# waffcloud/sitewhere

Hardware: AMD Instinct MI355X
Metric: device_events_per_sec (higher is better)
Workload: dtype fp64/int64 (event values as in the reference; no reduced precision)

## Files before the change

### csrc/hip/swblock.h

```cpp
#pragma once
#include <hip/hip_runtime.h>
#include <stdint.h>
#include "swengine.h"

typedef unsigned long long ull;

__device__ __forceinline__ uint32_t lane_id() { return threadIdx.x & 63; }

template <typename T>
__device__ __forceinline__ T wave_incl_scan(T v) {
  const uint32_t lane = lane_id();
#pragma unroll
  for (int d = 1; d < 64; d <<= 1) {
    const T t = __shfl_up(v, d, 64);
    if (lane >= (uint32_t)d) v += t;
  }
  return v;
}

template <typename T, int WAVES = 4>
__device__ __forceinline__ T block_excl_scan(T v, T* total, T* lds) {
  const uint32_t wid = threadIdx.x >> 6;
  const T inc = wave_incl_scan(v);
  if (lane_id() == 63) lds[wid] = inc;
  __syncthreads();
  if (threadIdx.x == 0) {
    T acc = 0;
    for (int w = 0; w < WAVES; ++w) { const T t = lds[w]; lds[w] = acc; acc += t; }
    lds[WAVES] = acc;
  }
  __syncthreads();
  const T res = inc - v + lds[wid];
  *total = lds[WAVES];
  __syncthreads();
  return res;
}

template <int WAVES = 4>
__device__ __forceinline__ uint32_t block_sum_prefix(const uint32_t* v, int64_t k, uint32_t* lds) {
  uint32_t s = 0;
  for (int64_t i = threadIdx.x; i < k; i += WAVES * 64) s += v[i];
  uint32_t tot;
  block_excl_scan<uint32_t, WAVES>(s, &tot, lds);
  return tot;
}

template <bool BLOCK_WORDS>
__device__ __forceinline__ void step_snapshot_write(SwStepSnapshot* rec, uint32_t t, const uint32_t* scalars,
                                                    const uint32_t* block_meta, const uint32_t* rej_cnt,
                                                    const uint32_t* n_carry, bool produced) {
  constexpr uint32_t BLOCK = offsetof(SwStepSnapshot, block_bytes) / 4, CARRY = offsetof(SwStepSnapshot, n_carry) / 4,
                     REJ = offsetof(SwStepSnapshot, rej_refs) / 4, PAD = offsetof(SwStepSnapshot, pad) / 4;
  static_assert(BLOCK == SW_SC_WORDS && CARRY == BLOCK + 6 && REJ == CARRY + 2 && PAD == REJ + 2, "word ladder");
  uint32_t* w = reinterpret_cast<uint32_t*>(rec);
  if (t < BLOCK) w[t] = produced ? scalars[t] : 0u;
  else if (t < CARRY) { if (BLOCK_WORDS) w[t] = (produced && block_meta) ? block_meta[t - BLOCK] : 0u; }
  else if (t == CARRY || t == CARRY + 1) w[t] = n_carry ? n_carry[t - CARRY] : 0u;
  else if (t == REJ || t == REJ + 1) w[t] = (produced && rej_cnt) ? rej_cnt[t - REJ] : 0u;
}

extern "C" int sw_radix_sort_u32(uint32_t* keys, uint32_t* vals, const uint32_t* n_ptr, int64_t cap, int bits, uint32_t* hist,
                      uint32_t* vals_final, hipStream_t s);
```

### csrc/hip/swgpu.hip

```cpp
#include <hip/hip_runtime.h>
#include <hsa/hsa.h>
#include <hsa/hsa_ext_amd.h>
#include <stdint.h>
#include "swtypes.h"
#include "swdecode.h"
#include "swengine.h"
#include "swseg.h"
#include "swblock.h"

#define BLK 256
#define WAVES (BLK / 64)
#define TILE_ITEMS 4
#define TILE (BLK * TILE_ITEMS)
#define MAX_GRID 2048
#define STAGE_BYTES (32 * 1024)
#define MAX_PROBE 4096

#ifndef SW_XCD_REMAP
#define SW_XCD_REMAP 0
#endif
__device__ __forceinline__ uint32_t sw_block_id() {
#if SW_XCD_REMAP
  const uint32_t nwg = gridDim.x, orig = blockIdx.x, x = orig % 8u, q = nwg / 8u, r = nwg % 8u;
  return (x < r ? x * (q + 1u) : r * (q + 1u) + (x - r) * q) + orig / 8u;
// ... 2167 lines not shown

int sw_reject_pack(const void* recs, const int32_t* rej_idx, const uint8_t* status, const uint32_t* scalars,
                   int64_t cap, void* out, uint8_t* out_st, hipStream_t s) {
  static_assert(sizeof(SwEventRec) == 80, "k_reject_pack copies 5 x 16 B per record");
  if (cap <= 0 || cap > 0xffffffffll / 5) return -1;
  k_reject_pack<<<512, 256, 0, s>>>(reinterpret_cast<const uint4*>(recs), rej_idx, status, scalars, (uint32_t)cap,
                                    reinterpret_cast<uint4*>(out), out_st);
  return (int)hipGetLastError();
}

int sw_stream_wait_event(hipStream_t s, hipEvent_t e) { return (int)hipStreamWaitEvent(s, e, 0); }
int sw_event_record(hipEvent_t e, hipStream_t s) { return (int)hipEventRecord(e, s); }
int sw_memcpy_h2d_async(void* dst, const void* src, int64_t n, hipStream_t s) {
  return n > 0 ? (int)hipMemcpyAsync(dst, src, (size_t)n, hipMemcpyHostToDevice, s) : 0;
}
int sw_memset_async(void* dst, int32_t v, int64_t n, hipStream_t s) {
  return n > 0 ? (int)hipMemsetAsync(dst, v, (size_t)n, s) : 0;
}

int sw_step_snapshot(const uint32_t* scalars, const uint32_t* seg_meta, const uint32_t* rej_cnt,
                     const uint32_t* n_carry, int32_t produced, SwStepSnapshot* host, hipStream_t s) {
  k_step_snapshot<<<1, 64, 0, s>>>(scalars, seg_meta, rej_cnt, n_carry, produced, host);
  return (int)hipGetLastError();
}

int sw_frame_varint(const uint8_t* lens, int64_t nbytes, int64_t n_msgs, uint32_t* msg_off, uint32_t raw_bytes,
                    uint32_t* tmp, int64_t tmp_len, hipStream_t s) {
  int64_t nt = (nbytes + TILE - 1) / TILE;
  if (nt < 1) nt = 1;
  if (2 * nt > tmp_len) return -2;
  if (nbytes <= 0 || n_msgs <= 0) return (int)hipMemsetAsync(msg_off, 0, sizeof(uint32_t) * (n_msgs + 1), s);
  uint32_t* tcnt = tmp;
  uint32_t* tlen = tmp + nt;
  k_vlen_tiles<<<(unsigned)nt, BLK, 0, s>>>(lens, nbytes, tcnt, tlen);
  k_vlen_apply<<<(unsigned)nt, BLK, 0, s>>>(lens, nbytes, tcnt, tlen, msg_off, n_msgs, raw_bytes);
  return (int)hipGetLastError();
}

int sw_phase_decode(const SwEngineArgs* ap, hipStream_t s) {
  const SwEngineArgs a = *ap;
  if (a.n_msgs <= 0) {
    k_decode_begin<<<1, 64, 0, s>>>(a);
    (void)hipMemsetAsync(a.n_recs, 0, sizeof(uint32_t), s);
    return (int)hipGetLastError();
  }
  const unsigned nb = (unsigned)((a.n_msgs + BLK - 1) / BLK);
  k_decode_count<<<nb, BLK, 0, s>>>(a.raw, a.msg_off, a.n_msgs, a.msg_cnt, a.msg_evoff, a);
  k_decode_emit<<<nb, BLK, 0, s>>>(a);
  if (a.world > 1) k_decode_end<<<1, 64, 0, s>>>(a);
  return (int)hipGetLastError();
}

int sw_phase_partition(const SwEngineArgs* ap, hipStream_t s) {
  const SwEngineArgs a = *ap;
  const int64_t ntiles = (a.carry_cap + a.rec_cap + TILE - 1) / TILE;
  if (a.world > 64 || ntiles * a.world > a.part_tmp_len || !a.carry || !a.n_carry || !a.spill || !a.n_spill ||
      a.carry == a.spill || !a.part_owner || !a.part_bytes || !a.part_meta || ntiles >= 0x7fffffff)
    return -3;
  if (a.send_str && (!a.part_len || !a.carry_spans || !a.carry_str || !a.spill_spans || !a.spill_str ||
                     a.carry_str == a.spill_str || a.carry_str_cap <= 0 || a.carry_str_cap > 0xffffffffll ||
                     a.str_cap > 0x7fffffffll))
    return -4;
  k_part_count<<<(unsigned)ntiles, BLK, 0, s>>>(a.carry, a.n_carry, a.recs, a.n_recs, (int)a.world, (int)a.rank,
                                                a.part_tmp, ntiles, a);
  int rc = launch_scan(a.part_tmp, ntiles * a.world, a.part_tmp + ntiles * a.world, nullptr, a.scan_tmp,
                       a.scan_tmp_len, s);
  if (rc) return rc;
  const uint32_t* toff = a.part_tmp + ntiles * a.world;
  k_part_cut<<<(unsigned)a.world, BLK, 0, s>>>(toff, a.part_tmp, ntiles, a.n_carry, a.n_recs, a);
  k_part_write<<<(unsigned)ntiles, BLK, 0, s>>>(a.carry, a.n_carry, a.recs, a.n_recs, (int)a.world, (int)a.rank, toff,
                                                a.part_tmp, ntiles, a.send, a.shuf_cap, a.spill, a.carry_cap, a);
  k_part_counts<<<1, 64, 0, s>>>(toff, a.part_tmp, ntiles, (int)a.world, a);
  return (int)hipGetLastError();
}

int sw_phase_unpack(const SwEngineArgs* ap, hipStream_t s) {
  const SwEngineArgs a = *ap;
  if (a.work_str && (a.str_cap & 15)) return -5;
  k_unpack<<<grid_for(a.rec_cap), BLK, 0, s>>>(a.recv, a.recv_cnt, (int)a.world, a.shuf_cap, a.work, a.n_work,
                                               a.rec_cap, a);
  return (int)hipGetLastError();
}

__global__ void k_cl_prep(const uint32_t* __restrict__ ok_idx, const uint32_t* __restrict__ n_ok,
                          const int32_t* __restrict__ ev_asg, uint32_t* __restrict__ keys, uint32_t* __restrict__ vals) {
  const uint32_t n = *n_ok;
  for (int64_t j = (int64_t)BID * BLK + threadIdx.x; j < n; j += (int64_t)gridDim.x * BLK) {
    const uint32_t i = ok_idx[j];
    keys[j] = (uint32_t)ev_asg[i];
    vals[j] = i;
  }
}

__global__ __launch_bounds__(BLK) void k_ff_add_rows(SwEngineArgs a, const SwEventRec* __restrict__ R,
                                                     const uint32_t* __restrict__ idx,
                                                     const uint32_t* __restrict__ n_ptr, uint32_t cap) {
  if (!a.dd_ff) return;
  const uint32_t n = *n_ptr < cap ? *n_ptr : cap;
  uint32_t* __restrict__ t = a.dd_ff;
  const int gens = (int)a.dd_ff_gens, g = (int)a.dd_ff_meta[0];
  const int64_t bmask = a.dd_ff_bmask;
  const uint32_t lane = threadIdx.x & 63u, sub = lane & 3u, grp = lane >> 2;
  const ull gmask = 0xfull << (4u * grp);
  const int64_t g0 = ((int64_t)BID * BLK + threadIdx.x) >> 2;
  const int64_t gstride = ((int64_t)gridDim.x * BLK) >> 2;
  uint32_t dropped = 0;
  for (int64_t base = g0 - grp; base < (int64_t)n; base += gstride) {
    const int64_t j = base + grp;
    ull h = 0ull;
    if (j < (int64_t)n) h = R[idx ? idx[j] : (uint32_t)j].alt_hash;
    const ull m = sw_ff_mix(h);
    const uint32_t fp = sw_ff_fp(m);
    int64_t b = (int64_t)sw_ff_bucket(m, bmask);
    bool pending = h != 0ull;
    for (int p = 0; p < 2 * SW_FF_MAX_PROBE && __any(pending); ++p) {
      uint32_t* sl = t + (b * gens + g) * SW_FF_SLOTS;
      uint4 v = make_uint4(1u, 1u, 1u, 1u);
      if (pending) v = reinterpret_cast<const uint4*>(sl)[sub];
      const bool hit = pending && (v.x == fp || v.y == fp || v.z == fp || v.w == fp);
      if (__ballot(hit) & gmask) pending = false;
      const bool zero = pending && (!v.x || !v.y || !v.z || !v.w);
      const ull zb = __ballot(zero) & gmask;
      bool ok = false;
      if (pending && zb && lane == (uint32_t)(__ffsll((long long)zb) - 1)) {
        const int k = !v.x ? 0 : !v.y ? 1 : !v.z ? 2 : 3;
        const uint32_t old = atomicCAS(&sl[4u * sub + (uint32_t)k], 0u, fp);
        ok = old == 0u || old == fp;
      }
      if (__ballot(ok) & gmask) pending = false;
      else if (pending && !zb) b = (b + 1) & bmask;
    }
    if (pending && sub == 0u) ++dropped;
  }
  if (dropped) atomicAdd((ull*)&a.dd_ff_meta[5], (ull)dropped);
}

int sw_phase_process(const SwEngineArgs* ap, uint32_t* scratch4, hipStream_t s) {
  const SwEngineArgs a = *ap;
  const int g = grid_for(a.rec_cap);
  const int64_t ntiles = (a.rec_cap + TILE - 1) / TILE;
  if (2 * ntiles > a.scan_tmp_len) return -4;
  if (a.dd_ff && (a.dd_ff_gens < 2 || a.dd_ff_gens > SW_FF_MAX_GENS || !a.dd_ff_meta || a.dd_ff_bmask < 0))
    return -6;
  if (a.n_mtests < 0 || (a.n_mtests > 0 && (!a.mtests || a.n_tests + a.n_mtests > ZONE_LDS_TESTS))) return -7;
  k_lookup<<<g, BLK, 0, s>>>(a);
  if (a.dd_ff) k_ff_probe<<<g, BLK, 0, s>>>(a);
  k_dedup_claim<<<g, BLK, 0, s>>>(a);
  k_cmp_count<<<(unsigned)ntiles, BLK, 0, s>>>(a.status, a.n_work, a.cmp_tmp, ntiles, (ull*)a.stats, a.work,
                                               (const ull*)a.dd_key, a.dd_mask, a.seq_base, a.dd_meta,
                                               a.dd_ff, a.dd_ff_bmask, (int)a.dd_ff_gens, a.work_str ? -1 : (int)a.rank);
  k_cmp_write<<<(unsigned)ntiles, BLK, 0, s>>>(a.status, a.n_work, a.cmp_tmp, ntiles, a.ok_idx, a.rej_idx, a.n_ok,
                                               a.n_rej);
  int rc = 0;
  if (a.cl_bits > 0) {
    k_cl_prep<<<g, BLK, 0, s>>>(a.ok_idx, a.n_ok, a.ev_asg, a.cl_keys, a.cl_vals);
    rc = sw_radix_sort_u32(a.cl_keys, a.cl_vals, a.n_ok, a.rec_cap, (int)a.cl_bits, a.cl_hist, a.ok_idx, s);
    if (rc < 0) return rc;
  }
  const SwStrRef* wsp = a.world > 1 ? a.work_spans : a.spans;
  k_persist<<<g, BLK, 0, s>>>(a, a.work, a.ok_idx, a.ev_dev, a.ev_asg, a.n_ok, (uint32_t)a.rec_cap, wsp, nullptr);
  if (a.dd_ff) k_ff_add_rows<<<g, BLK, 0, s>>>(a, a.work, a.ok_idx, a.n_ok, (uint32_t)a.rec_cap);
  k_state_p2<<<g, BLK, 0, s>>>(a, a.n_ok, (uint32_t)a.rec_cap, nullptr);
  uint32_t* n_rule = scratch4;
  if (a.n_tests + a.n_mtests > 0) {
    const int64_t otiles = (a.rec_cap + TILE - 1) / TILE;
    ull* zmask = (ull*)a.zmask;
    uint32_t* ztile = a.ztile;
    if (a.n_tests > 0) {
      const size_t vtx_bytes = zone_vtx_in_lds(a) ? (size_t)a.n_zone_vtx * 2 * sizeof(double) : 0;
      k_zone_mask<<<(unsigned)otiles, BLK, vtx_bytes, s>>>(a, zmask, ztile);
    }
    if (a.n_mtests > 0) k_mx_mask<<<(unsigned)otiles, BLK, 0, s>>>(a, zmask, ztile, a.n_tests > 0 ? 0 : 1);
    k_zone_emit<<<(unsigned)otiles, BLK, 0, s>>>(a, zmask, ztile, n_rule);
  } else {
    k_gen_clamp<<<1, 64, 0, s>>>(a, n_rule);
  }
  k_presence<<<grid_for(a.n_asg), BLK, 0, s>>>(a);
  const int gg = grid_for(a.gen_cap);
  const uint32_t gcap = (uint32_t)a.gen_cap;
  k_intern_insert_list<<<gg, BLK, 0, s>>>(a.gen, a.n_gen, (ull*)a.nm_key, a.nm_id, a.nm_counter, a.nm_mask, gcap);
  k_persist<<<gg, BLK, 0, s>>>(a, a.gen, nullptr, a.gen_dev, a.gen_asg, a.n_gen, gcap, nullptr, a.n_ok);
  if (a.dd_ff) k_ff_add_rows<<<gg, BLK, 0, s>>>(a, a.gen, nullptr, a.n_gen, gcap);
  k_state_p2<<<gg, BLK, 0, s>>>(a, a.n_gen, gcap, a.n_ok);
  k_step_end<<<1, 64, 0, s>>>(a, n_rule);
  return (int)hipGetLastError();
}

__global__ void k_set_step_params(SwStepParams* sp, int64_t now_ms, int64_t batch_seq, int64_t presence_ms,
                                  SwOutRec* out, void* aux, int64_t raw_bytes) {
  if (threadIdx.x == 0 && BID == 0) {
    sp->now_ms = now_ms; sp->batch_seq = batch_seq; sp->presence_missing_ms = presence_ms; sp->out = out;
    sp->aux = aux; sp->raw_bytes = raw_bytes;
  }
}

__global__ void k_ff_add(uint32_t* t, int64_t bmask, int gens, int g, int64_t* meta, const ull* __restrict__ h,
                         int64_t n) {
  uint32_t dropped = 0;
  for (int64_t i = (int64_t)BID * BLK + threadIdx.x; i < n; i += (int64_t)gridDim.x * BLK)
    if (h[i] && !ff_add(t, bmask, gens, g, h[i])) ++dropped;
  if (dropped) atomicAdd((ull*)&meta[5], (ull)dropped);
}

__global__ void k_ff_clear(uint32_t* t, int64_t bmask, int gens, int g) { ff_clear_gen(t, bmask, gens, g); }

int sw_ff_add(void* tab, int64_t bmask, int64_t gens, int64_t gen, void* meta, const void* hashes, int64_t n,
              hipStream_t s) {
  if (n <= 0) return 0;
  if (gens < 2 || gens > SW_FF_MAX_GENS || gen < 0 || gen >= gens) return -2;
  const int64_t g = (n + BLK - 1) / BLK;
  k_ff_add<<<(unsigned)(g < 4096 ? g : 4096), BLK, 0, s>>>((uint32_t*)tab, bmask, (int)gens, (int)gen,
                                                          (int64_t*)meta, (const ull*)hashes, n);
  return (int)hipGetLastError();
}

int sw_ff_clear(void* tab, int64_t bmask, int64_t gens, int64_t g, hipStream_t s) {
  if (gens < 2 || gens > SW_FF_MAX_GENS || g < 0 || g >= gens) return -2;
  const int64_t nb = (bmask + 1) * 4;
  const int64_t gr = (nb + BLK - 1) / BLK;
  k_ff_clear<<<(unsigned)(gr < 8192 ? gr : 8192), BLK, 0, s>>>((uint32_t*)tab, bmask, (int)gens, (int)g);
  return (int)hipGetLastError();
}

int sw_set_step_params(SwStepParams* sp, int64_t now_ms, int64_t batch_seq, int64_t presence_ms, void* out,
                       void* aux, int64_t raw_bytes, hipStream_t s) {
  k_set_step_params<<<1, 64, 0, s>>>(sp, now_ms, batch_seq, presence_ms, (SwOutRec*)out, aux, raw_bytes);
  return (int)hipGetLastError();
}

int sw_graph_capture_process(const SwEngineArgs* ap, uint32_t* scratch4, int32_t with_unpack, hipStream_t s,
                             void** exec_out) {
  hipGraph_t g = nullptr;
  hipError_t e = hipStreamBeginCapture(s, hipStreamCaptureModeThreadLocal);
  if (e != hipSuccess) return 5000 + (int)e;
  int rc = 0;
  if (with_unpack) rc = sw_phase_unpack(ap, s);
  if (!rc) rc = sw_phase_process(ap, scratch4, s);
  e = hipStreamEndCapture(s, &g);
  if (rc) { if (g) (void)hipGraphDestroy(g); return rc; }
// ... 308 lines not shown
```

### csrc/hip/swindex.hip

```cpp
#include <hip/hip_runtime.h>
#include <stdint.h>
#include "swindex.h"
#include "swseg.h"
#include "swtypes.h"
#include "swblock.h"

#define RS_BLK 256
#define RS_ITEMS 16
#define RS_TILE (RS_BLK * RS_ITEMS)
#define RS_WAVES (RS_BLK / 64)

struct RsState {
  uint32_t* hist;
  uint32_t* off;
  uint32_t* tot;
};

__device__ __host__ __forceinline__ int64_t rs_tiles(int64_t cap) {
  const int64_t t = (cap + RS_TILE - 1) / RS_TILE;
  return t < 1 ? 1 : t;
}
__device__ __host__ __forceinline__ RsState rs_state(uint32_t* st, int64_t cap) {
  RsState r;
  const int64_t tiles = rs_tiles(cap);
  r.hist = st;
  r.off = st + tiles * 256;
  r.tot = r.off + tiles * 256;
  return r;
}

__global__ __launch_bounds__(RS_BLK) void k_rs_count(const uint32_t* __restrict__ keys, const uint32_t* __restrict__ n_ptr,
                                                     int shift, uint32_t mask, uint32_t* st_words, int64_t cap) {
  __shared__ uint32_t h[256];
  const RsState st = rs_state(st_words, cap);
  const uint32_t n = *n_ptr;
  const int64_t base = (int64_t)blockIdx.x * RS_TILE;
  if (base >= (int64_t)n) return;
  h[threadIdx.x] = 0;
  __syncthreads();
#pragma unroll
  for (int k = 0; k < RS_ITEMS; ++k) {
    const int64_t i = base + (int64_t)k * RS_BLK + threadIdx.x;
    if (i < (int64_t)n) atomicAdd(&h[(keys[i] >> shift) & mask], 1u);
  }
  __syncthreads();
  st.hist[(int64_t)blockIdx.x * 256 + threadIdx.x] = h[threadIdx.x];
}

__global__ __launch_bounds__(RS_BLK) void k_rs_offsets(const uint32_t* __restrict__ n_ptr, uint32_t* st_words, int64_t cap) {
  __shared__ uint32_t red[RS_WAVES + 1];
  const RsState st = rs_state(st_words, cap);
  const uint32_t n = *n_ptr;
  const int64_t ntiles = ((int64_t)n + RS_TILE - 1) / RS_TILE;
  const uint32_t d = blockIdx.x;
  uint32_t run = 0;
  for (int64_t t0 = 0; t0 < ntiles; t0 += RS_BLK) {
    const int64_t t = t0 + threadIdx.x;
    const uint32_t v = t < ntiles ? st.hist[t * 256 + d] : 0u;
    uint32_t tot;
    const uint32_t pre = block_excl_scan(v, &tot, red);
    if (t < ntiles) st.off[t * 256 + d] = run + pre;
    run += tot;
  }
  if (threadIdx.x == 0) st.tot[d] = run;
}

struct RsLds {
  uint32_t sk[RS_TILE];
  uint32_t sv[RS_TILE];
  uint32_t wc[RS_WAVES][256];
  uint32_t ls[256];
  uint32_t run[256];
  uint32_t gb[256];
  uint32_t red[RS_WAVES + 1];
};

__global__ __launch_bounds__(RS_BLK) void k_rs_scatter(const uint32_t* __restrict__ kin, const uint32_t* __restrict__ vin,
                                                       uint32_t* __restrict__ kout, uint32_t* __restrict__ vout,
                                                       const uint32_t* __restrict__ n_ptr, int shift, int dbits,
                                                       uint32_t* st_words, int64_t cap) {
  __shared__ RsLds L;
  const RsState st = rs_state(st_words, cap);
  const uint32_t n = *n_ptr;
  const int64_t tile = blockIdx.x;
  const int64_t base = tile * RS_TILE;
  if (base >= (int64_t)n) return;
  const uint32_t t = threadIdx.x, lane = lane_id(), wid = t >> 6;
  const uint32_t mask = (1u << dbits) - 1u;
  uint32_t K[RS_ITEMS], V[RS_ITEMS];
#pragma unroll
  for (int k = 0; k < RS_ITEMS; ++k) {
    const int64_t i = base + (int64_t)k * RS_BLK + t;
    const bool ok = i < (int64_t)n;
    K[k] = ok ? kin[i] : 0u;
    V[k] = ok ? vin[i] : 0u;
  }
  uint32_t gtot, ctot;
  const uint32_t gpre = block_excl_scan(t <= mask ? st.tot[t] : 0u, &gtot, L.red);
  const uint32_t c = t <= mask ? st.hist[tile * 256 + t] : 0u;
  L.ls[t] = block_excl_scan(c, &ctot, L.red);
  L.gb[t] = gpre + (t <= mask ? st.off[tile * 256 + t] : 0u);
  L.run[t] = 0;
#pragma unroll
  for (int w = 0; w < RS_WAVES; ++w) L.wc[w][t] = 0;
  __syncthreads();
  const ull lt = (1ull << lane) - 1ull;
#pragma unroll
  for (int k = 0; k < RS_ITEMS; ++k) {
    const int64_t i = base + (int64_t)k * RS_BLK + t;
    const bool valid = i < (int64_t)n;
    const uint32_t d = (K[k] >> shift) & mask;
    ull peers = __ballot(valid);
    for (int b = 0; b < dbits; ++b) {
      const bool bit = (d >> b) & 1u;
      const ull m = __ballot(valid && bit);
      peers &= bit ? m : ~m;
    }
    const uint32_t rank = (uint32_t)__popcll(peers & lt);
    if (valid && rank == 0) L.wc[wid][d] = (uint32_t)__popcll(peers);
    __syncthreads();
    if (valid) {
      uint32_t pos = L.ls[d] + L.run[d] + rank;
      for (uint32_t w = 0; w < wid; ++w) pos += L.wc[w][d];
      L.sk[pos] = K[k];
      L.sv[pos] = V[k];
    }
    __syncthreads();
    uint32_t add = 0;
#pragma unroll
    for (int w = 0; w < RS_WAVES; ++w) { add += L.wc[w][t]; L.wc[w][t] = 0; }
    L.run[t] += add;
    __syncthreads();
  }
  const uint32_t m = (uint32_t)(((int64_t)n - base) < RS_TILE ? (int64_t)n - base : RS_TILE);
  for (uint32_t i = t; i < m; i += RS_BLK) {
    const uint32_t key = L.sk[i];
    const uint32_t d = (key >> shift) & mask;
    const uint32_t pos = L.gb[d] + (i - L.ls[d]);
    kout[pos] = key;
    vout[pos] = L.sv[i];
  }
}

extern "C" {

int64_t sw_radix_tmp_words(int64_t cap) { return 2 * 256 * rs_tiles(cap) + 256 + 8; }

int sw_radix_sort_u32(uint32_t* keys, uint32_t* vals, const uint32_t* n_ptr, int64_t cap, int bits, uint32_t* state,
                      uint32_t* vals_final, hipStream_t s) {
  if (bits <= 0) return 0;
  if (bits > 32) bits = 32;
  const unsigned grid = (unsigned)rs_tiles(cap);
  int cur = 0;
  const int passes = (bits + 7) / 8;
  for (int p = 0; p < passes; ++p) {
    const int db = bits - 8 * p < 8 ? bits - 8 * p : 8;
    const uint32_t mask = (1u << db) - 1u;
    const bool last = p == passes - 1;
    uint32_t* vo = (last && vals_final) ? vals_final : vals + (int64_t)(1 - cur) * cap;
    k_rs_count<<<grid, RS_BLK, 0, s>>>(keys + (int64_t)cur * cap, n_ptr, 8 * p, mask, state, cap);
    k_rs_offsets<<<1u << db, RS_BLK, 0, s>>>(n_ptr, state, cap);
    k_rs_scatter<<<grid, RS_BLK, 0, s>>>(keys + (int64_t)cur * cap, vals + (int64_t)cur * cap,
                                         keys + (int64_t)(1 - cur) * cap, vo, n_ptr, 8 * p, db, state, cap);
    cur = 1 - cur;
  }
  const int rc = (int)hipGetLastError();
  return rc ? -rc : cur;
}

}

struct SwIxScratch {
  SwIxHdr h;
  uint64_t tstart;
  uint64_t cs;
  uint32_t n_alt;
  uint32_t n_chunks[SIX_DIMS];
  uint32_t scans_done;
  uint32_t finish_done;
  uint32_t err;
  uint32_t n_sort;
  uint32_t unsorted;
};

#define IX_CHUNK 1024
#define IX_PREP_BLK 1024
#define IX_LDS_KEYS 16384

struct SwIxArgs {
  const SwOutRec* rows;
  const SwSegAux* aux;
  const uint8_t* raw;
  const int64_t* cursor;
  const uint64_t* s_alt;
  int64_t store_cap;
  const int4* asg_ctx;
  int64_t n_asg;
  uint8_t* out;
  int64_t out_cap;
  uint64_t* seg_state;
  int64_t max_pages;
  SwStepSnapshot* snap_host;
  int32_t nk[SIX_DIMS];
  int32_t nk_off[SIX_DIMS];
  int32_t nk_total;
  int32_t lds_all;
  int32_t groups;
  uint32_t* skeys;
  uint32_t* svals;
  uint32_t* rstate;
  uint32_t* whist;
  uint32_t* ccnt;
  uint32_t* coff;
  uint32_t* ckeys;
  uint4* krec;
  uint32_t* cmap;
  int64_t mcap;
  uint32_t* cdone;
  uint32_t* brow;
  int64_t* bdate;
  int64_t* part;
  int64_t pcap;
  SwIxScratch* sc;
  int64_t cap;
  uint64_t* stamps;
};

#define IX_PART_WORDS (2 + 2 * SIX_HEADS)

struct IxKeyRec {
  uint32_t key, cnt, off, hoff, pch, chunk0, pad0, pad1;
};

__device__ __forceinline__ int64_t ix_rows(const SwIxArgs& a) {
  const int64_t n = a.cursor[0] - a.cursor[1];
  return n < 0 ? 0 : (n > a.cap ? a.cap : n);
}
__device__ __forceinline__ int32_t ix_ctx(const SwIxArgs& a, int32_t asg, int d) {
  if (asg < 0 || asg >= a.n_asg) return -1;
  const int4 c = a.asg_ctx[asg];
  return d == 0 ? c.y : d == 1 ? c.z : c.w;
}
__device__ __forceinline__ bool ix_encoder_failed(const SwIxArgs& a) {
  return a.seg_state[a.max_pages + SEG_ST_ERRORS] != 0;
}
__device__ __forceinline__ void ix_range(const SwIxArgs& a, int64_t n, int64_t* r0, int64_t* r1) {
  const int64_t per = ((n + a.groups - 1) / a.groups + 63) & ~63ll;
  *r0 = (int64_t)blockIdx.x * per;
  *r1 = *r0 + per < n ? *r0 + per : n;
}
// ... 578 lines not shown
  sc->cs = 0;
  sc->n_alt = 0;
  sc->unsorted = 0;
  sc->scans_done = 0;
  sc->finish_done = 0;
  sc->err = 0;
}

static int64_t ix_mcap(int64_t cap) { return cap / IX_CHUNK + SIX_KEYS + 1; }

extern "C" {

static int64_t ix_pcap(int64_t cap) { return 2 * (cap / IX_CHUNK) + 2; }

int64_t sw_seg_index_groups(int64_t cap) {
  const int64_t g = (cap + 4095) / 4096;
  return g < 1 ? 1 : (g > 256 ? 256 : g);
}


int64_t sw_seg_index_scratch_words(int64_t cap, int64_t nk_total) {
  const int64_t g = sw_seg_index_groups(cap);
  return 4 * cap + sw_radix_tmp_words(cap) + g * (nk_total > 0 ? nk_total : 1) + 4ll * SIX_DIMS * SIX_KEYS +
         SIX_DIMS * ix_mcap(cap) + 4 + 8ll * SIX_DIMS * SIX_KEYS +
         SIX_DIMS * cap + 2 * SIX_DIMS * cap + 2 * SIX_DIMS * ix_pcap(cap) * IX_PART_WORDS +
         (int64_t)((sizeof(SwIxScratch) + 15) / 4) + 16;
}

int64_t sw_seg_index_max_bytes(int64_t rows) { return (int64_t)six_max_bytes((uint64_t)rows); }


int sw_seg_index(const void* rows, const void* aux, const uint8_t* raw, const int64_t* cursor, const uint64_t* s_alt,
                 int64_t store_cap, const void* asg_ctx, int64_t n_asg, const int32_t* nk, uint8_t* out,
                 int64_t out_cap, uint64_t* seg_state, int64_t max_pages, SwStepSnapshot* snap_host, uint32_t* scratch,
                 int64_t cap, uint64_t* stamps, hipStream_t s) {
  SwIxArgs a;
  a.stamps = stamps;
  a.rows = (const SwOutRec*)rows;
  a.aux = (const SwSegAux*)aux;
  a.raw = raw;
  a.cursor = cursor;
  a.s_alt = s_alt;
  a.store_cap = store_cap;
  a.asg_ctx = (const int4*)asg_ctx;
  a.n_asg = n_asg;
  a.out = out;
  a.out_cap = out_cap;
  a.seg_state = seg_state;
  a.max_pages = max_pages;
  a.snap_host = snap_host;
  int32_t tot = 0;
  for (int d = 0; d < SIX_DIMS; ++d) {
    a.nk[d] = nk[d] > SIX_KEYS ? -1 : nk[d];
    a.nk_off[d] = tot;
    tot += a.nk[d] > 0 ? a.nk[d] : 0;
  }
  a.nk_total = tot > 0 ? tot : 1;
  a.lds_all = tot <= IX_LDS_KEYS ? 1 : 0;
  a.groups = (int32_t)sw_seg_index_groups(cap);
  uint32_t* p = scratch;
  a.skeys = p; p += 2 * cap;
  a.svals = p; p += 2 * cap;
  a.rstate = p; p += sw_radix_tmp_words(cap);
  a.whist = p; p += (int64_t)a.groups * a.nk_total;
  a.ccnt = p; p += (int64_t)SIX_DIMS * SIX_KEYS;
  a.coff = p; p += (int64_t)SIX_DIMS * SIX_KEYS;
  a.ckeys = p; p += (int64_t)SIX_DIMS * SIX_KEYS;
  a.cdone = p; p += (int64_t)SIX_DIMS * SIX_KEYS;
  a.mcap = ix_mcap(cap);
  a.cmap = p; p += SIX_DIMS * a.mcap;
  p += (4 - ((uintptr_t)p & 15) / 4) & 3;
  a.krec = reinterpret_cast<uint4*>(p); p += 8ll * SIX_DIMS * SIX_KEYS;
  a.brow = p; p += SIX_DIMS * cap;
  p += ((uintptr_t)p & 7) ? 1 : 0;
  a.bdate = reinterpret_cast<int64_t*>(p); p += 2 * SIX_DIMS * cap;
  a.pcap = ix_pcap(cap);
  a.part = reinterpret_cast<int64_t*>(p); p += 2 * SIX_DIMS * a.pcap * IX_PART_WORDS;
  p += ((uintptr_t)p & 7) ? 1 : 0;
  a.sc = reinterpret_cast<SwIxScratch*>(p);
  a.cap = cap;
  k_ix_prep<<<(unsigned)a.groups, IX_PREP_BLK, 0, s>>>(a);
  const int rc = sw_radix_sort_u32(a.skeys, a.svals, &a.sc->n_sort, cap, SIX_ALT_SORT_BITS + 1, a.rstate, nullptr, s);
  if (rc < 0) return -rc;
  k_ix_colscan<<<(unsigned)((a.nk_total + 255) / 256), 256, 0, s>>>(a);
  k_ix_scan<<<SIX_DIMS, IX_SCAN_BLK, 0, s>>>(a);
  k_ix_scatter<<<(unsigned)a.groups, IX_PREP_BLK, 0, s>>>(a);
  k_ix_write<<<IX_WRITE_WGS, IX_WBLK, 0, s>>>(a);
  k_ix_heads<<<IX_WRITE_WGS, IX_WBLK, 0, s>>>(a);
  k_ix_merge<<<64, IX_WBLK, 0, s>>>(a);
  k_ix_finish<<<256, IX_WBLK, 0, s>>>(a);
  return (int)hipGetLastError();
}

}
```

### sitewhere_amd/_native.py

```python
from __future__ import annotations

import ctypes
import os
import shutil
import subprocess
import threading
from pathlib import Path

ROOT = Path(__file__).resolve().parent.parent
LIB_DIR = Path(__file__).resolve().parent / "_lib"
CSRC = ROOT / "csrc"
GPU_ARCH = os.environ.get("SW_GPU_ARCH", "gfx950")

_NATIVE_SRC = [CSRC / "native" / "swnative.cpp", CSRC / "native" / "swcpuengine.cpp", CSRC / "native" / "swseg.cpp",
               CSRC / "native" / "swindex.cpp", CSRC / "native" / "swroute.cpp", CSRC / "native" / "swsandbox.cpp", CSRC / "native" / "swjson.cpp",
               CSRC / "native" / "swrowjson.cpp"]
_GPU_SRC = [CSRC / "hip" / "swgpu.hip", CSRC / "hip" / "swseg.hip", CSRC / "hip" / "swindex.hip"]
_HEADERS = sorted((CSRC / "include").glob("*.h")) + sorted((CSRC / "hip").glob("*.h"))

_lock = threading.Lock()
_native = None
_gpu = None


# ... 207 lines not shown
_native_gil = None


def native_gil():
    global _native_gil
    if _native_gil is not None:
        return _native_gil
    lib0 = native()
    with _lock:
        if _native_gil is None:
            lib = ctypes.PyDLL(lib0._name)
            P = c_void_p
            _proto(lib, "swlog_topic", c_int32, P, c_char_p, c_int32)
            _proto(lib, "swlog_partitions", c_int32, P, c_int32)
            _proto(lib, "swlog_append_batch", c_int64, P, c_int32, c_int32, P, P, P, P, P, c_int64)
            _proto(lib, "swlog_append_routed", c_int64, P, P, P, c_int64, P, P, c_int64, P)
            _proto(lib, "swlog_append", c_int64, P, c_int32, c_int32, P, c_int64, P, c_int64, c_int64)
            _proto(lib, "swlog_end_offset", c_int64, P, c_int32, c_int32)
            _proto(lib, "swlog_begin_offset", c_int64, P, c_int32, c_int32)
            _proto(lib, "swlog_read", c_int64, P, c_int32, c_int32, c_int64, c_int64, P, c_int64, P)
            _proto(lib, "swlog_commit", c_int32, P, c_char_p, c_int32, c_int32, c_int64)
            _proto(lib, "swlog_committed", c_int64, P, c_char_p, c_int32, c_int32)
            _proto(lib, "swlog_append_external", c_int64, P, c_int32, c_int32, P, c_int64, c_int64, c_int64,
                   c_int64)
            _proto(lib, "swlog_view", c_int32, P, c_int32, c_int32, c_int64, P, P, P)
            _proto(lib, "swlog_hold", c_int32, P, c_int32, c_int32, c_int64)
            _proto(lib, "swlog_take_released", c_int64, P, P, c_int64)
            _proto(lib, "sw_partition_for_key", c_int32, c_char_p, c_int32, c_int32)
            _native_gil = lib
    return _native_gil


def gpu():
    global _gpu
    if _gpu is not None:
        return _gpu
    import torch

    with _lock:
        if _gpu is not None:
            return _gpu
        override = os.environ.get("SW_GPU_LIB")
        path = Path(override) if override else LIB_DIR / "libswgpu.so"
        if not override and _stale(path, _GPU_SRC):
            build_gpu()
        lib = ctypes.CDLL(str(path))
        P = c_void_p
        _proto(lib, "sw_phase_decode", c_int32, P, P)
        _proto(lib, "sw_phase_partition", c_int32, P, P)
        _proto(lib, "sw_phase_unpack", c_int32, P, P)
        _proto(lib, "sw_phase_process", c_int32, P, P, P)
        _proto(lib, "sw_pip_batch", c_int32, P, c_int64, P, P, c_int64, P, P)
        _proto(lib, "sw_store_filter", c_int32, P, c_int32, P, c_int64, P, P)
        _proto(lib, "sw_store_series_count", c_int32, P, P, P, P)
        _proto(lib, "sw_store_series", c_int32, P, P, P, c_int64, P, P, c_int64, P, P, P, P, P)
        _proto(lib, "sw_store_near", c_int32, P, P, P, c_int64, P, P)
        _proto(lib, "sw_store_zone", c_int32, P, P, c_int64, P, P)
        _proto(lib, "sw_store_grid", c_int32, P, P, P, P)
        _proto(lib, "sw_grid_lds_cells", c_int64, c_int64)
        _proto(lib, "sw_store_rank", c_int32, P, P, P, P, P, P)
        _proto(lib, "sw_rank_lds_keys", c_int64, c_int64)
        _proto(lib, "sw_rank_combine", c_int32, c_int32)
        _proto(lib, "sw_scan_u32", c_int32, P, c_int64, P, P, P, c_int64, P)
        _proto(lib, "sw_state_lookup", c_int32, P, c_int64, c_int32, c_int32, P, P, P)
        _proto(lib, "sw_abi_sizes", c_int32, P)
        _proto(lib, "sw_host_alloc", c_int32, c_int64, P, P)
        _proto(lib, "sw_host_free", c_int32, P)
        _proto(lib, "sw_push_out", c_int32, P, P, P, c_int64, c_int32, P)
        _proto(lib, "sw_copy_d2h", c_int32, P, P, c_int64, P)
        _proto(lib, "sw_sdma_copy", c_int32, P, P, c_int64, c_int32, ctypes.POINTER(ctypes.c_uint64))
        _proto(lib, "sw_sdma_h2d", c_int32, P, P, c_int64, c_int32, ctypes.POINTER(ctypes.c_uint64))
        _proto(lib, "sw_frame_varint", c_int32, P, c_int64, c_int64, P, ctypes.c_uint32, P, c_int64, P)
        _proto(lib, "sw_set_step_params", c_int32, P, c_int64, c_int64, c_int64, P, P, c_int64, P)
        _proto(lib, "sw_graph_capture_process", c_int32, P, P, c_int32, P, ctypes.POINTER(ctypes.c_void_p))
        _proto(lib, "sw_graph_launch", c_int32, P, P)
        _proto(lib, "sw_graph_destroy", c_int32, P)
        _proto(lib, "sw_sdma_wait", c_int32, c_uint64)
        _proto(lib, "sw_seg_encode", c_int32, P, P, P, P, P, c_int64, P, c_int64, P)
        _proto(lib, "sw_seg_encode_stamped", c_int32, P, P, P, P, P, c_int64, P, c_int64, P, P)
        _proto(lib, "sw_seg_encode_snap", c_int32, P, P, P, P, P, c_int64, P, c_int64, P, P, P, P, P)
        _proto(lib, "sw_seg_aux", c_int32, P, P, P, P, P, c_int64, P, P, c_int64, P)
        _proto(lib, "sw_radix_tmp_words", c_int64, c_int64)
        _proto(lib, "sw_radix_sort_u32", c_int32, P, P, P, c_int64, c_int32, P, P, P)
        _proto(lib, "sw_seg_index_scratch_words", c_int64, c_int64, c_int64)
        _proto(lib, "sw_seg_index_max_bytes", c_int64, c_int64)
        _proto(lib, "sw_seg_index", c_int32, P, P, P, P, P, c_int64, P, c_int64, P, P, c_int64, P, c_int64, P, P,
               c_int64, P, P)
        _proto(lib, "sw_ff_add", c_int32, P, c_int64, c_int64, c_int64, P, P, c_int64, P)
        _proto(lib, "sw_ff_clear", c_int32, P, c_int64, c_int64, c_int64, P)
        _proto(lib, "sw_reject_refs", c_int32, P, P, P, c_int64, P, P, c_int64, P, c_int64, P)
        _proto(lib, "sw_step_snapshot", c_int32, P, P, P, P, c_int32, P, P)
        _proto(lib, "sw_reject_pack", c_int32, P, P, P, P, c_int64, P, P, P)
        _proto(lib, "sw_stream_wait_event", c_int32, P, P)
        _proto(lib, "sw_event_record", c_int32, P, P)
        _proto(lib, "sw_memcpy_h2d_async", c_int32, P, P, c_int64, P)
        _proto(lib, "sw_memset_async", c_int32, P, c_int32, c_int64, P)
        _gpu = lib
        return lib


_GPU_BLOCKING = {"sw_sdma_wait"}
_gpu_gil = None


class _GilBound:

    def __init__(self, cdll):
        self._c = cdll
        self._p = ctypes.PyDLL(cdll._name)

    def __getattr__(self, name):
        f = getattr(self._c, name)
        if name in _GPU_BLOCKING or name.startswith("_"):
            return f
        g = getattr(self._p, name)
        g.restype, g.argtypes = f.restype, f.argtypes
        setattr(self, name, g)
        return g


def gpu_gil():
    global _gpu_gil
    if _gpu_gil is None:
        lib = gpu()
        with _lock:
            if _gpu_gil is None:
                _gpu_gil = _GilBound(lib)
    return _gpu_gil


def gpu_library_path() -> Path:
    return LIB_DIR / "libswgpu.so"
```

Before: 561.1 million.

## Restructure radix sort with gather-fused first pass and wave-local ranking

Removes the separate key-gather kernel by fusing the ev_asg gather into the first radix count and scatter passes, and drops key writes on the final pass. The scatter kernel now ranks items per wave with LDS counters instead of block-wide syncs on every item, and packs global and local offsets into one 64-bit scan. Digit width is configurable up to 8 bits split evenly across passes, and the offsets kernel scans several digits per block. The index sort caller now follows the returned buffer parity. This adds complexity and relies on the packed 16-bit local count fitting within a tile.

```diff
diff --git a/csrc/hip/swblock.h b/csrc/hip/swblock.h
--- a/csrc/hip/swblock.h
+++ b/csrc/hip/swblock.h
@@ -61,3 +61,6 @@
 
 extern "C" int sw_radix_sort_u32(uint32_t* keys, uint32_t* vals, const uint32_t* n_ptr, int64_t cap, int bits, uint32_t* hist,
                       uint32_t* vals_final, hipStream_t s);
+extern "C" int sw_radix_sort_gather_u32(const uint32_t* idx, const uint32_t* src, uint32_t* keys, uint32_t* vals,
+                                        const uint32_t* n_ptr, int64_t cap, int bits, uint32_t* state,
+                                        uint32_t* vals_final, hipStream_t s);
diff --git a/csrc/hip/swgpu.hip b/csrc/hip/swgpu.hip
--- a/csrc/hip/swgpu.hip
+++ b/csrc/hip/swgpu.hip
@@ -2273,16 +2273,6 @@
   return (int)hipGetLastError();
 }
 
-__global__ void k_cl_prep(const uint32_t* __restrict__ ok_idx, const uint32_t* __restrict__ n_ok,
-                          const int32_t* __restrict__ ev_asg, uint32_t* __restrict__ keys, uint32_t* __restrict__ vals) {
-  const uint32_t n = *n_ok;
-  for (int64_t j = (int64_t)BID * BLK + threadIdx.x; j < n; j += (int64_t)gridDim.x * BLK) {
-    const uint32_t i = ok_idx[j];
-    keys[j] = (uint32_t)ev_asg[i];
-    vals[j] = i;
-  }
-}
-
 __global__ __launch_bounds__(BLK) void k_ff_add_rows(SwEngineArgs a, const SwEventRec* __restrict__ R,
                                                      const uint32_t* __restrict__ idx,
                                                      const uint32_t* __restrict__ n_ptr, uint32_t cap) {
@@ -2344,8 +2334,8 @@
                                                a.n_rej);
   int rc = 0;
   if (a.cl_bits > 0) {
-    k_cl_prep<<<g, BLK, 0, s>>>(a.ok_idx, a.n_ok, a.ev_asg, a.cl_keys, a.cl_vals);
-    rc = sw_radix_sort_u32(a.cl_keys, a.cl_vals, a.n_ok, a.rec_cap, (int)a.cl_bits, a.cl_hist, a.ok_idx, s);
+    rc = sw_radix_sort_gather_u32(a.ok_idx, (const uint32_t*)a.ev_asg, a.cl_keys, a.cl_vals, a.n_ok, a.rec_cap,
+                                  (int)a.cl_bits, a.cl_hist, a.ok_idx, s);
     if (rc < 0) return rc;
   }
   const SwStrRef* wsp = a.world > 1 ? a.work_spans : a.spans;
diff --git a/csrc/hip/swindex.hip b/csrc/hip/swindex.hip
--- a/csrc/hip/swindex.hip
+++ b/csrc/hip/swindex.hip
@@ -6,13 +6,24 @@
 #include "swblock.h"
 
 #define RS_BLK 256
-#define RS_ITEMS 16
+#ifndef RS_ITEMS
+#define RS_ITEMS 8
+#endif
+#ifndef RS_MAXW
+#define RS_MAXW 8
+#endif
 #define RS_TILE (RS_BLK * RS_ITEMS)
 #define RS_WAVES (RS_BLK / 64)
+#define RS_RUN (RS_TILE / RS_WAVES)
+#define RS_D (1 << RS_MAXW)
+#define RS_PER (RS_D > RS_BLK ? RS_D / RS_BLK : 1)
+#define RS_OD 4
+#define RS_OT (RS_BLK / RS_OD)
+#define RS_OC 16
+static_assert(RS_MAXW >= 1 && RS_MAXW <= 12 && RS_TILE < 65536 && RS_RUN % 64 == 0, "radix sort geometry");
 
 struct RsState {
-  uint32_t* hist;
-  uint32_t* off;
+  uint32_t* cnt;
   uint32_t* tot;
 };
 
@@ -22,63 +33,103 @@
 }
 __device__ __host__ __forceinline__ RsState rs_state(uint32_t* st, int64_t cap) {
   RsState r;
-  const int64_t tiles = rs_tiles(cap);
-  r.hist = st;
-  r.off = st + tiles * 256;
-  r.tot = r.off + tiles * 256;
+  r.cnt = st;
+  r.tot = st + rs_tiles(cap) * RS_D;
   return r;
 }
 
-__global__ __launch_bounds__(RS_BLK) void k_rs_count(const uint32_t* __restrict__ keys, const uint32_t* __restrict__ n_ptr,
-                                                     int shift, uint32_t mask, uint32_t* st_words, int64_t cap) {
-  __shared__ uint32_t h[256];
+template <bool GATHER>
+__global__ __launch_bounds__(RS_BLK) void k_rs_count(const uint32_t* __restrict__ kin, const uint32_t* __restrict__ vin,
+                                                     const uint32_t* __restrict__ src, const uint32_t* __restrict__ n_ptr,
+                                                     int shift, int dbits, uint32_t* st_words, int64_t cap) {
+  __shared__ uint32_t h[RS_D];
   const RsState st = rs_state(st_words, cap);
   const uint32_t n = *n_ptr;
   const int64_t base = (int64_t)blockIdx.x * RS_TILE;
   if (base >= (int64_t)n) return;
-  h[threadIdx.x] = 0;
-  __syncthreads();
+  const uint32_t nd = 1u << dbits, mask = nd - 1u;
+  for (uint32_t d = threadIdx.x; d < nd; d += RS_BLK) h[d] = 0;
+  __syncthreads();
+  uint32_t K[RS_ITEMS];
 #pragma unroll
   for (int k = 0; k < RS_ITEMS; ++k) {
     const int64_t i = base + (int64_t)k * RS_BLK + threadIdx.x;
-    if (i < (int64_t)n) atomicAdd(&h[(keys[i] >> shift) & mask], 1u);
-  }
-  __syncthreads();
-  st.hist[(int64_t)blockIdx.x * 256 + threadIdx.x] = h[threadIdx.x];
-}
-
-__global__ __launch_bounds__(RS_BLK) void k_rs_offsets(const uint32_t* __restrict__ n_ptr, uint32_t* st_words, int64_t cap) {
-  __shared__ uint32_t red[RS_WAVES + 1];
+    K[k] = i < (int64_t)n ? (GATHER ? vin[i] : kin[i]) : 0u;
+  }
+  if (GATHER) {
+#pragma unroll
+    for (int k = 0; k < RS_ITEMS; ++k) K[k] = base + (int64_t)k * RS_BLK + threadIdx.x < (int64_t)n ? src[K[k]] : 0u;
+  }
+#pragma unroll
+  for (int k = 0; k < RS_ITEMS; ++k)
+    if (base + (int64_t)k * RS_BLK + threadIdx.x < (int64_t)n) atomicAdd(&h[(K[k] >> shift) & mask], 1u);
+  __syncthreads();
+  for (uint32_t d = threadIdx.x; d < nd; d += RS_BLK) st.cnt[(int64_t)blockIdx.x * nd + d] = h[d];
+}
+
+__global__ __launch_bounds__(RS_BLK) void k_rs_offsets(const uint32_t* __restrict__ n_ptr, uint32_t* st_words, int64_t cap,
+                                                       int dbits) {
+  __shared__ uint32_t part[RS_WAVES][RS_OD];
   const RsState st = rs_state(st_words, cap);
   const uint32_t n = *n_ptr;
   const int64_t ntiles = ((int64_t)n + RS_TILE - 1) / RS_TILE;
-  const uint32_t d = blockIdx.x;
-  uint32_t run = 0;
-  for (int64_t t0 = 0; t0 < ntiles; t0 += RS_BLK) {
-    const int64_t t = t0 + threadIdx.x;
-    const uint32_t v = t < ntiles ? st.hist[t * 256 + d] : 0u;
-    uint32_t tot;
-    const uint32_t pre = block_excl_scan(v, &tot, red);
-    if (t < ntiles) st.off[t * 256 + d] = run + pre;
-    run += tot;
-  }
-  if (threadIdx.x == 0) st.tot[d] = run;
+  const uint32_t nd = 1u << dbits;
+  const uint32_t t = threadIdx.x, lane = lane_id(), wid = t >> 6;
+  const uint32_t dl = t % RS_OD, tl = t / RS_OD, d = blockIdx.x * RS_OD + dl;
+  const int64_t chunk = (ntiles + RS_OT - 1) / RS_OT;
+  const int64_t t0 = tl * chunk < ntiles ? tl * chunk : ntiles, t1 = t0 + chunk < ntiles ? t0 + chunk : ntiles;
+  const bool live = d < nd, regs = chunk <= RS_OC;
+  uint32_t* col = st.cnt + d;
+  uint32_t c[RS_OC];
+  uint32_t sum = 0;
+  if (regs) {
+#pragma unroll
+    for (int k = 0; k < RS_OC; ++k) {
+      c[k] = (live && t0 + k < t1) ? col[(t0 + k) * nd] : 0u;
+      sum += c[k];
+    }
+  } else if (live) {
+    for (int64_t i = t0; i < t1; ++i) sum += col[i * nd];
+  }
+  uint32_t inc = sum;
+#pragma unroll
+  for (uint32_t o = RS_OD; o < 64; o <<= 1) {
+    const uint32_t v = __shfl_up(inc, o, 64);
+    if (lane >= o) inc += v;
+  }
+  if (lane >= 64 - RS_OD) part[wid][dl] = inc;
+  __syncthreads();
+  uint32_t run = inc - sum;
+  for (uint32_t w = 0; w < wid; ++w) run += part[w][dl];
+  if (!live) return;
+  if (tl == RS_OT - 1) st.tot[d] = run + sum;
+  if (regs) {
+#pragma unroll
+    for (int k = 0; k < RS_OC; ++k) {
+      if (t0 + k < t1) col[(t0 + k) * nd] = run;
+      run += c[k];
+    }
+  } else {
+    for (int64_t i = t0; i < t1; ++i) {
+      const uint32_t v = col[i * nd];
+      col[i * nd] = run;
+      run += v;
+    }
+  }
 }
 
 struct RsLds {
   uint32_t sk[RS_TILE];
   uint32_t sv[RS_TILE];
-  uint32_t wc[RS_WAVES][256];
-  uint32_t ls[256];
-  uint32_t run[256];
-  uint32_t gb[256];
-  uint32_t red[RS_WAVES + 1];
+  uint32_t wc[RS_WAVES][RS_D];
+  ull red[RS_WAVES + 1];
 };
 
+template <bool GATHER>
 __global__ __launch_bounds__(RS_BLK) void k_rs_scatter(const uint32_t* __restrict__ kin, const uint32_t* __restrict__ vin,
-                                                       uint32_t* __restrict__ kout, uint32_t* __restrict__ vout,
-                                                       const uint32_t* __restrict__ n_ptr, int shift, int dbits,
-                                                       uint32_t* st_words, int64_t cap) {
+                                                       const uint32_t* __restrict__ src, uint32_t* __restrict__ kout,
+                                                       uint32_t* __restrict__ vout, const uint32_t* __restrict__ n_ptr,
+                                                       int shift, int dbits, uint32_t* st_words, int64_t cap) {
   __shared__ RsLds L;
   const RsState st = rs_state(st_words, cap);
   const uint32_t n = *n_ptr;
@@ -86,29 +137,33 @@
   const int64_t base = tile * RS_TILE;
   if (base >= (int64_t)n) return;
   const uint32_t t = threadIdx.x, lane = lane_id(), wid = t >> 6;
-  const uint32_t mask = (1u << dbits) - 1u;
-  uint32_t K[RS_ITEMS], V[RS_ITEMS];
+  const uint32_t nd = 1u << dbits, mask = nd - 1u;
+  const int64_t wbase = base + (int64_t)wid * RS_RUN + lane;
+  uint32_t K[RS_ITEMS], V[RS_ITEMS], R[RS_ITEMS];
 #pragma unroll
   for (int k = 0; k < RS_ITEMS; ++k) {
-    const int64_t i = base + (int64_t)k * RS_BLK + t;
+    const int64_t i = wbase + k * 64;
     const bool ok = i < (int64_t)n;
-    K[k] = ok ? kin[i] : 0u;
     V[k] = ok ? vin[i] : 0u;
-  }
-  uint32_t gtot, ctot;
-  const uint32_t gpre = block_excl_scan(t <= mask ? st.tot[t] : 0u, &gtot, L.red);
-  const uint32_t c = t <= mask ? st.hist[tile * 256 + t] : 0u;
-  L.ls[t] = block_excl_scan(c, &ctot, L.red);
-  L.gb[t] = gpre + (t <= mask ? st.off[tile * 256 + t] : 0u);
-  L.run[t] = 0;
-#pragma unroll
-  for (int w = 0; w < RS_WAVES; ++w) L.wc[w][t] = 0;
-  __syncthreads();
+    K[k] = ok ? (GATHER ? src[V[k]] : kin[i]) : 0u;
+  }
+  const uint32_t per = nd > RS_BLK ? nd / RS_BLK : 1u;
+  uint32_t T[RS_PER], C[RS_PER];
+#pragma unroll
+  for (uint32_t j = 0; j < RS_PER; ++j) {
+    const uint32_t d = t * per + j;
+    const bool ok = j < per && d < nd;
+    T[j] = ok ? st.tot[d] : 0u;
+    C[j] = ok ? st.cnt[tile * nd + d] : 0u;
+  }
+  uint32_t* mine = L.wc[wid];
+  for (uint32_t d = lane; d < nd; d += 64) mine[d] = 0;
+  __builtin_amdgcn_fence(__ATOMIC_ACQ_REL, "wavefront");
+  __builtin_amdgcn_wave_barrier();
   const ull lt = (1ull << lane) - 1ull;
 #pragma unroll
   for (int k = 0; k < RS_ITEMS; ++k) {
-    const int64_t i = base + (int64_t)k * RS_BLK + t;
-    const bool valid = i < (int64_t)n;
+    const bool valid = wbase + k * 64 < (int64_t)n;
     const uint32_t d = (K[k] >> shift) & mask;
     ull peers = __ballot(valid);
     for (int b = 0; b < dbits; ++b) {
@@ -116,56 +171,120 @@
       const ull m = __ballot(valid && bit);
       peers &= bit ? m : ~m;
     }
-    const uint32_t rank = (uint32_t)__popcll(peers & lt);
-    if (valid && rank == 0) L.wc[wid][d] = (uint32_t)__popcll(peers);
-    __syncthreads();
-    if (valid) {
-      uint32_t pos = L.ls[d] + L.run[d] + rank;
-      for (uint32_t w = 0; w < wid; ++w) pos += L.wc[w][d];
+    const uint32_t r = (valid ? mine[d] : 0u) + (uint32_t)__popcll(peers & lt);
+    R[k] = r;
+    if (valid && (peers >> lane) == 1ull) mine[d] = r + 1u;
+    __builtin_amdgcn_fence(__ATOMIC_ACQ_REL, "wavefront");
+    __builtin_amdgcn_wave_barrier();
+  }
+  __syncthreads();
+  ull v = 0;
+#pragma unroll
+  for (uint32_t j = 0; j < RS_PER; ++j) {
+    const uint32_t d = t * per + j;
+    if (j < per && d < nd) {
+      uint32_t c = 0;
+#pragma unroll
+      for (int w = 0; w < RS_WAVES; ++w) c += L.wc[w][d];
+      v += ((ull)T[j] << 16) + c;
+    }
+  }
+  ull vtot;
+  const ull pre = block_excl_scan<ull, RS_WAVES>(v, &vtot, L.red);
+  uint32_t ls = (uint32_t)(pre & 0xffffu), gs = (uint32_t)(pre >> 16);
+  uint32_t delta[RS_PER];
+#pragma unroll
+  for (uint32_t j = 0; j < RS_PER; ++j) {
+    const uint32_t d = t * per + j;
+    delta[j] = 0;
+    if (j < per && d < nd) {
+      delta[j] = gs + C[j] - ls;
+      gs += T[j];
+#pragma unroll
+      for (int w = 0; w < RS_WAVES; ++w) {
+        const uint32_t c = L.wc[w][d];
+        L.wc[w][d] = ls;
+        ls += c;
+      }
+    }
+  }
+  __syncthreads();
+#pragma unroll
+  for (int k = 0; k < RS_ITEMS; ++k) {
+    if (wbase + k * 64 < (int64_t)n) {
+      const uint32_t pos = mine[(K[k] >> shift) & mask] + R[k];
       L.sk[pos] = K[k];
       L.sv[pos] = V[k];
     }
-    __syncthreads();
-    uint32_t add = 0;
-#pragma unroll
-    for (int w = 0; w < RS_WAVES; ++w) { add += L.wc[w][t]; L.wc[w][t] = 0; }
-    L.run[t] += add;
-    __syncthreads();
-  }
+  }
+  __syncthreads();
+#pragma unroll
+  for (uint32_t j = 0; j < RS_PER; ++j) {
+    const uint32_t d = t * per + j;
+    if (j < per && d < nd) L.wc[0][d] = delta[j];
+  }
+  __syncthreads();
   const uint32_t m = (uint32_t)(((int64_t)n - base) < RS_TILE ? (int64_t)n - base : RS_TILE);
   for (uint32_t i = t; i < m; i += RS_BLK) {
     const uint32_t key = L.sk[i];
-    const uint32_t d = (key >> shift) & mask;
-    const uint32_t pos = L.gb[d] + (i - L.ls[d]);
-    kout[pos] = key;
+    const uint32_t pos = i + L.wc[0][(key >> shift) & mask];
+    if (kout) kout[pos] = key;
     vout[pos] = L.sv[i];
   }
 }
 
 extern "C" {
 
-int64_t sw_radix_tmp_words(int64_t cap) { return 2 * 256 * rs_tiles(cap) + 256 + 8; }
+int64_t sw_radix_tmp_words(int64_t cap) { return RS_D * rs_tiles(cap) + RS_D + 8; }
+
+}
+
+static int rs_sort(const uint32_t* idx, const uint32_t* src, uint32_t* keys, uint32_t* vals, const uint32_t* n_ptr,
+                   int64_t cap, int bits, int min_passes, uint32_t* state, uint32_t* vals_final, bool drop_keys,
+                   hipStream_t s) {
+  if (bits > 32) bits = 32;
+  const unsigned grid = (unsigned)rs_tiles(cap);
+  int passes = (bits + RS_MAXW - 1) / RS_MAXW;
+  if (passes < min_passes) passes = min_passes;
+  int cur = 0, shift = 0;
+  for (int p = 0; p < passes; ++p) {
+    const int db = bits / passes + (p < bits % passes ? 1 : 0);
+    const bool last = p == passes - 1;
+    const uint32_t* ki = keys + (int64_t)cur * cap;
+    const uint32_t* vi = vals + (int64_t)cur * cap;
+    uint32_t* ko = (last && drop_keys) ? nullptr : keys + (int64_t)(1 - cur) * cap;
+    uint32_t* vo = (last && vals_final) ? vals_final : vals + (int64_t)(1 - cur) * cap;
+    if (p == 0 && idx) {
+      k_rs_count<true><<<grid, RS_BLK, 0, s>>>(nullptr, idx, src, n_ptr, shift, db, state, cap);
+      k_rs_offsets<<<((1u << db) + RS_OD - 1) / RS_OD, RS_BLK, 0, s>>>(n_ptr, state, cap, db);
+      k_rs_scatter<true><<<grid, RS_BLK, 0, s>>>(nullptr, idx, src, ko, vo, n_ptr, shift, db, state, cap);
+    } else {
+      k_rs_count<false><<<grid, RS_BLK, 0, s>>>(ki, vi, nullptr, n_ptr, shift, db, state, cap);
+      k_rs_offsets<<<((1u << db) + RS_OD - 1) / RS_OD, RS_BLK, 0, s>>>(n_ptr, state, cap, db);
+      k_rs_scatter<false><<<grid, RS_BLK, 0, s>>>(ki, vi, nullptr, ko, vo, n_ptr, shift, db, state, cap);
+    }
+    shift += db;
+    cur = 1 - cur;
+  }
+  const int rc = (int)hipGetLastError();
+  return rc ? -rc : cur;
+}
+
+extern "C" {
 
 int sw_radix_sort_u32(uint32_t* keys, uint32_t* vals, const uint32_t* n_ptr, int64_t cap, int bits, uint32_t* state,
                       uint32_t* vals_final, hipStream_t s) {
   if (bits <= 0) return 0;
-  if (bits > 32) bits = 32;
-  const unsigned grid = (unsigned)rs_tiles(cap);
-  int cur = 0;
-  const int passes = (bits + 7) / 8;
-  for (int p = 0; p < passes; ++p) {
-    const int db = bits - 8 * p < 8 ? bits - 8 * p : 8;
-    const uint32_t mask = (1u << db) - 1u;
-    const bool last = p == passes - 1;
-    uint32_t* vo = (last && vals_final) ? vals_final : vals + (int64_t)(1 - cur) * cap;
-    k_rs_count<<<grid, RS_BLK, 0, s>>>(keys + (int64_t)cur * cap, n_ptr, 8 * p, mask, state, cap);
-    k_rs_offsets<<<1u << db, RS_BLK, 0, s>>>(n_ptr, state, cap);
-    k_rs_scatter<<<grid, RS_BLK, 0, s>>>(keys + (int64_t)cur * cap, vals + (int64_t)cur * cap,
-                                         keys + (int64_t)(1 - cur) * cap, vo, n_ptr, 8 * p, db, state, cap);
-    cur = 1 - cur;
-  }
-  const int rc = (int)hipGetLastError();
-  return rc ? -rc : cur;
+  return rs_sort(nullptr, nullptr, keys, vals, n_ptr, cap, bits, 1, state, vals_final, false, s);
+}
+
+int sw_radix_sort_gather_u32(const uint32_t* idx, const uint32_t* src, uint32_t* keys, uint32_t* vals,
+                             const uint32_t* n_ptr, int64_t cap, int bits, uint32_t* state, uint32_t* vals_final,
+                             hipStream_t s) {
+  if (!idx || !src || !vals_final) return -(int)hipErrorInvalidValue;
+  if (bits <= 0) return idx == vals_final ? 0 : -(int)hipErrorInvalidValue;
+  const int rc = rs_sort(idx, src, keys, vals, n_ptr, cap, bits, idx == vals_final ? 2 : 1, state, vals_final, true, s);
+  return rc < 0 ? rc : 0;
 }
 
 }
@@ -910,6 +1029,8 @@
   k_ix_prep<<<(unsigned)a.groups, IX_PREP_BLK, 0, s>>>(a);
   const int rc = sw_radix_sort_u32(a.skeys, a.svals, &a.sc->n_sort, cap, SIX_ALT_SORT_BITS + 1, a.rstate, nullptr, s);
   if (rc < 0) return -rc;
+  a.skeys += (int64_t)rc * cap;
+  a.svals += (int64_t)rc * cap;
   k_ix_colscan<<<(unsigned)((a.nk_total + 255) / 256), 256, 0, s>>>(a);
   k_ix_scan<<<SIX_DIMS, IX_SCAN_BLK, 0, s>>>(a);
   k_ix_scatter<<<(unsigned)a.groups, IX_PREP_BLK, 0, s>>>(a);
diff --git a/sitewhere_amd/_native.py b/sitewhere_amd/_native.py
--- a/sitewhere_amd/_native.py
+++ b/sitewhere_amd/_native.py
@@ -313,6 +313,7 @@
         _proto(lib, "sw_seg_aux", c_int32, P, P, P, P, P, c_int64, P, P, c_int64, P)
         _proto(lib, "sw_radix_tmp_words", c_int64, c_int64)
         _proto(lib, "sw_radix_sort_u32", c_int32, P, P, P, c_int64, c_int32, P, P, P)
+        _proto(lib, "sw_radix_sort_gather_u32", c_int32, P, P, P, P, P, c_int64, c_int32, P, P, P)
         _proto(lib, "sw_seg_index_scratch_words", c_int64, c_int64, c_int64)
         _proto(lib, "sw_seg_index_max_bytes", c_int64, c_int64)
         _proto(lib, "sw_seg_index", c_int32, P, P, P, P, P, c_int64, P, c_int64, P, P, c_int64, P, c_int64, P, P,
```

After: 538.8 million. 4.0% lower.
